# Santhosh-Sathyamurthy/cfd-simulations

Hardware: AMD Instinct MI355X
Metric: Gcell-updates/s on pressure-Poisson Jacobi; achieved HBM GB/s vs peak (higher is better)
Workload: dtype f32; 1 GPU; jacobi3d_7pt_1024x1024x1024_f32; decomposition=z-slab, halo=none, kernel_variant=0, waves=0, zchunk=0, temporal_blocking=0, tb_rows=0, rhs_workspace=True

## Files before the change

cfd-simulations_amd/csrc/jacobi3d_tbr.hip:

```cpp
#include <type_traits>

#include "internal.hpp"

namespace cfd {

namespace {

typedef float gv4g __attribute__((ext_vector_type(4)));
typedef const __attribute__((address_space(1))) gv4g *gcv4p;
typedef __attribute__((address_space(1))) gv4g *gv4p;
__device__ inline float4 ldg4(const float *p) {
    const gv4g v = *(gcv4p)p;
    return make_float4(v.x, v.y, v.z, v.w);
}
__device__ inline void stg4(float *p, float4 v) { *(gv4p)p = gv4g{v.x, v.y, v.z, v.w}; }
__device__ inline float4 lds4(const float *p) { return *reinterpret_cast<const float4 *>(p); }
__device__ inline void sts4(float *p, float4 v) { *reinterpret_cast<float4 *>(p) = v; }

typedef float gv4f __attribute__((ext_vector_type(4)));
typedef __attribute__((address_space(3))) void lds_void;
typedef __attribute__((address_space(3))) float lfloat;
typedef __attribute__((address_space(3))) gv4f lgv4f;
__device__ inline uint32_t lds_addr(const void *p) { return (uint32_t)(uintptr_t)(const lds_void *)p; }
__device__ inline lfloat *lds_ptr(uint32_t a) { return (lfloat *)(uintptr_t)a; }
__device__ inline float4 lds4l(const lfloat *p) {
    const gv4f v = *(const lgv4f *)p;
    return make_float4(v.x, v.y, v.z, v.w);
}
__device__ inline void sts4l(lfloat *p, float4 v) { *(lgv4f *)p = gv4f{v.x, v.y, v.z, v.w}; }
__device__ inline __amdgpu_buffer_rsrc_t plane_rsrc(const float *base, int p, int nz, size_t plane) {
    const bool in = p >= 0 && p <= nz - 1;
    return __builtin_amdgcn_make_buffer_rsrc(const_cast<float *>(in ? base + (size_t)p * plane : base),
                                             (short)0, in ? (int)(plane * sizeof(float)) : 0, 0x00020000);
}
constexpr int kStoreNt = 2;
#ifndef CFD_TBR_LB
#define CFD_TBR_LB 1
#endif
#ifndef CFD_TBR_XW
#define CFD_TBR_XW 1
#endif
#ifndef CFD_TBR_SD
#define CFD_TBR_SD 1
#endif
#ifndef CFD_TBR_T0S
#define CFD_TBR_T0S 1
#endif
#ifndef CFD_TBR_EARLY
#define CFD_TBR_EARLY 1
#endif


__device__ inline float4 ldb4(__amdgpu_buffer_rsrc_t r, uint32_t byte_ofs) {
    const gv4f v = __builtin_amdgcn_raw_buffer_load_b128(r, (int)byte_ofs, 0, 0);
    return make_float4(v.x, v.y, v.z, v.w);
}
__device__ inline v4i32 plane_rsrc4(const float *base, int p, int nz, size_t plane) {
    const bool in = p >= 0 && p <= nz - 1;
    const unsigned long long b = (unsigned long long)(in ? base + (size_t)p * plane : base);
    v4i32 r;
    r.x = __builtin_amdgcn_readfirstlane((int)(unsigned)b);
    r.y = __builtin_amdgcn_readfirstlane((int)((unsigned)(b >> 32) & 0xffffu));
    r.z = __builtin_amdgcn_readfirstlane(in ? (int)(plane * sizeof(float)) : 0);
    r.w = 0x00020000;
    return r;
}
__device__ inline void lds_barrier() { asm volatile("s_waitcnt lgkmcnt(0)\n\ts_barrier" ::: "memory"); }
enum { kJacobi = 0, kRbgs = 1 };
constexpr int sl3(int v) { return ((v % 3) + 3) % 3; }
constexpr int slk(int v, int k) { return ((v % k) + k) % k; }

struct TbrArgs {
    const float *in;
    float *out;
    const float *div;
    int nz, ny, nx, nseg, ntile_y, zb, ze, zchunk, fixed_lo, fixed_hi;
    float h2, dt;
    float cx, cy, cz, cd, dt_inv, tol;
    int zoff;
    int h0;
    float *maxc;
    int rollback;
    int nhalf;
    const int *count;
    int lag;
    float *rhs_out;
    int xbw;
    unsigned long long *trace;
};
constexpr int kTraceStep0 = 200, kTraceSteps = 64;
__device__ inline void trace_mark(unsigned long long *tr, int wave, int step, int e) {
#ifdef CFD_TBR_TRACE
    const int k = step - kTraceStep0;
    if (tr && blockIdx.x == 0 && (threadIdx.x & 63) == 0 && k >= 0 && k < kTraceSteps)
        tr[((size_t)wave * kTraceSteps + k) * 5 + e] = __builtin_readcyclecounter();
#else
    (void)tr;
    (void)wave;
    (void)step;
    (void)e;
#endif
}
enum { kFirstRhs = 1, kFirstZero = 2 };

template <int MODE, bool PRE, bool PK = false>
__device__ inline float4 level4(float4 c, float wl, float er, float4 N, float4 S, float4 U,
                                float4 D, float4 d, int x, int nx, bool upd, const TbrArgs &a,
                                int par, bool own, float &chg) {
    if (!upd) return c;
    if (MODE == kRbgs) {
        typedef float v2f __attribute__((ext_vector_type(2)));
        const bool hi = (par & 1) != 0;
        const v2f C = hi ? v2f{c.y, c.w} : v2f{c.x, c.z};
        const v2f E = hi ? v2f{c.z, er} : v2f{c.y, c.w};
        const v2f Wv = hi ? v2f{c.x, c.z} : v2f{wl, c.y};
        const v2f Nv = hi ? v2f{N.y, N.w} : v2f{N.x, N.z};
        const v2f Sv = hi ? v2f{S.y, S.w} : v2f{S.x, S.z};
        const v2f Uv = hi ? v2f{U.y, U.w} : v2f{U.x, U.z};
        const v2f Dv = hi ? v2f{D.y, D.w} : v2f{D.x, D.z};
        const v2f Rv = hi ? v2f{d.y, d.w} : v2f{d.x, d.z};
        const v2f rhs = -Rv * a.dt_inv;
        const v2f p = a.cx * (E + Wv);
        const v2f q = a.cy * (Nv + Sv);
        const v2f r = a.cz * (Uv + Dv);
        v2f o = (((p + q) + r) - rhs) * a.cd;
        const int x0 = x + (hi ? 1 : 0);
        o.x = (x0 != 0 && x0 != nx - 1) ? o.x : C.x;
        o.y = (x0 + 2 != nx - 1) ? o.y : C.y;
        if (own) {
            chg = fmaxf(chg, fabsf(o.x - C.x));
            chg = fmaxf(chg, fabsf(o.y - C.y));
        }
        return hi ? make_float4(c.x, o.x, c.z, o.y) : make_float4(o.x, c.y, o.y, c.w);
    }
    if constexpr (!PK) {
        float o[4];
        const float cv[4] = {c.x, c.y, c.z, c.w};
        const float nv[4] = {N.x, N.y, N.z, N.w};
        const float sv[4] = {S.x, S.y, S.z, S.w};
        const float uv[4] = {U.x, U.y, U.z, U.w};
        const float dv[4] = {D.x, D.y, D.z, D.w};
        const float rv[4] = {d.x, d.y, d.z, d.w};
#pragma unroll
        for (int k = 0; k < 4; ++k) {
            const float E = k < 3 ? cv[k + 1] : er;
            const float Wv = k > 0 ? cv[k - 1] : wl;
            float s = E + Wv;
            s = s + nv[k];
            s = s + sv[k];
            s = s + uv[k];
            s = s + dv[k];
            const float rhs = PRE ? rv[k] : (a.h2 * rv[k]) / a.dt;
            const int xk = x + k;
            o[k] = (xk != 0 && xk != nx - 1) ? (1.0f / 6.0f) * (s - rhs) : cv[k];
    }
    return make_float4(o[0], o[1], o[2], o[3]);
    }
    typedef float v2 __attribute__((ext_vector_type(2)));
    const v2 mid = {c.y, c.z};
    v2 s01 = mid + v2{wl, c.x};
    v2 s23 = v2{c.w, er} + mid;
    s01 = s01 + v2{N.x, N.y};
    s23 = s23 + v2{N.z, N.w};
    s01 = s01 + v2{S.x, S.y};
    s23 = s23 + v2{S.z, S.w};
    s01 = s01 + v2{U.x, U.y};
    s23 = s23 + v2{U.z, U.w};
    s01 = s01 + v2{D.x, D.y};
    s23 = s23 + v2{D.z, D.w};
    v2 r01 = {d.x, d.y}, r23 = {d.z, d.w};
    if constexpr (!PRE) {
        r01 = (a.h2 * r01) / a.dt;
        r23 = (a.h2 * r23) / a.dt;
    }
    v2 o01 = (1.0f / 6.0f) * (s01 - r01);
    v2 o23 = (1.0f / 6.0f) * (s23 - r23);
    o01.x = x != 0 ? o01.x : c.x;
    o23.y = x + 3 != nx - 1 ? o23.y : c.w;
    return make_float4(o01.x, o01.y, o23.x, o23.y);
}

typedef float v2f_t __attribute__((ext_vector_type(2)));
__device__ inline v2f_t pick2(float4 f, int h) { return h ? v2f_t{f.y, f.w} : v2f_t{f.x, f.z}; }
__device__ inline float4 join2(v2f_t a, v2f_t b, int h) {
    return h ? make_float4(b.x, a.x, b.y, a.y) : make_float4(a.x, b.x, a.y, b.y);
}
struct P4 {
    v2f_t e, o;
};
__device__ inline v2f_t pick2(const P4 &f, int h) { return h ? f.o : f.e; }
__device__ inline P4 split4(float4 f) { return P4{v2f_t{f.x, f.z}, v2f_t{f.y, f.w}}; }

#ifndef CFD_TBR_Q64
#define CFD_TBR_Q64 1
#endif
struct Q4 {
    unsigned long long lo, hi;
};
__device__ inline Q4 q4_of(float4 f) {
    return Q4{__builtin_bit_cast(unsigned long long, v2f_t{f.x, f.y}),
              __builtin_bit_cast(unsigned long long, v2f_t{f.z, f.w})};
}
__device__ inline float4 f4_of(const Q4 &q) {
    const v2f_t a = __builtin_bit_cast(v2f_t, q.lo), b = __builtin_bit_cast(v2f_t, q.hi);
    return make_float4(a.x, a.y, b.x, b.y);
}
[[maybe_unused]] __device__ inline float4 f4_of(float4 f) { return f; }
__device__ inline const P4 &f4_of(const P4 &p) { return p; }
__device__ inline P4 ldsp(const float *p) { return P4{v2f_t{p[0], p[2]}, v2f_t{p[1], p[3]}}; }
__device__ inline void sts4s(float *row, int lane, float4 v) {
    *reinterpret_cast<v2f_t *>(row + 4 + 2 * lane) = v2f_t{v.x, v.z};
    *reinterpret_cast<v2f_t *>(row + 132 + 2 * lane) = v2f_t{v.y, v.w};
}
__device__ inline void sts4s(float *row, int lane, const P4 &v) {
    *reinterpret_cast<v2f_t *>(row + 4 + 2 * lane) = v.e;
    *reinterpret_cast<v2f_t *>(row + 132 + 2 * lane) = v.o;
}
constexpr int kPairRow = 132;
__device__ inline v2f_t lds2s(const float *row, int lane, int h) {
    return *reinterpret_cast<const v2f_t *>(row + 4 + 128 * h + 2 * lane);
}
struct GsPk {
    v2f_t cx, cy, cz, cd, ndt;
};
__device__ inline GsPk gs_pk(const TbrArgs &a) {
    GsPk k{v2f_t{a.cx, a.cx}, v2f_t{a.cy, a.cy}, v2f_t{a.cz, a.cz}, v2f_t{a.cd, a.cd},
           v2f_t{-a.dt_inv, -a.dt_inv}};
    asm volatile("" : "+v"(k.cx), "+v"(k.cy), "+v"(k.cz), "+v"(k.cd), "+v"(k.ndt));
    return k;
}
__device__ inline v2f_t level2(v2f_t C, v2f_t O, float wl, float er, v2f_t N, v2f_t S, v2f_t U, v2f_t D,
                               v2f_t rhs, int h, int x, int nx, bool upd, const GsPk &a, bool own,
                               float &chg) {
    if (!upd) return C;
    const v2f_t E = h ? v2f_t{O.y, er} : v2f_t{O.x, O.y};
    const v2f_t W = h ? v2f_t{O.x, O.y} : v2f_t{wl, O.x};
    const v2f_t p = a.cx * (E + W);
    const v2f_t q = a.cy * (N + S);
    const v2f_t r = a.cz * (U + D);
    v2f_t o = (((p + q) + r) - rhs) * a.cd;
    const int x0 = x + h;
    if (h == 0) o.x = x0 != 0 ? o.x : C.x;
    if (h == 1) o.y = x0 + 2 != nx - 1 ? o.y : C.y;
    if (own) {
        chg = fmaxf(chg, fabsf(o.x - C.x));
        chg = fmaxf(chg, fabsf(o.y - C.y));
    }
    return o;
}

}

template <int K, int NWR, int RPW, bool PRE, int PD, int MODE, int F, bool SPLIT, bool PT, bool T0S = false>
__device__ __forceinline__ void tbr_halo_wave(const TbrArgs a, float *smem, int z0, int z1, int y0, int xs,
                                              int zl, float *slots = nullptr) {
    constexpr int NR = NWR * RPW + 2;
    constexpr int RS = 264, RS2 = kPairRow;
    int t0 = 0;
    auto T = [&](int l, int r) -> float * {
        if (T0S && l == 0) return slots + t0 + r * RS;
        int base = 0;
#pragma unroll
        for (int m = T0S ? 1 : 0; m < K; ++m)
            if (m < l) base += (NR - 2 * m) * (PT && m ? RS2 : RS);
        return smem + base + (r - l) * (PT && l ? RS2 : RS);
    };
    const int nz = a.nz, ny = a.ny, nx = a.nx;
    const int lane = threadIdx.x & 63;
    const int x = xs + 4 * lane;
    const bool xin = x < nx;
    const size_t plane = (size_t)ny * nx;
    const int zs = z0 - K + 1;
    auto P = [&](int p) { return a.in + (size_t)p * plane; };
    auto fixedp = [&](int p) { return (p == a.zb - 1 && a.fixed_lo) || (p == a.ze && a.fixed_hi); };
    const float4 z4 = make_float4(0.f, 0.f, 0.f, 0.f);
// ... 139 lines not shown
        return t;
    }();
    __shared__ __attribute__((aligned(16))) float smem[TOTAL > 0 ? TOTAL : 4];
    __shared__ __attribute__((aligned(16))) float slots[T0S ? 3 * SLOT : 4];
    constexpr int SR_ = NR - 2;
    constexpr int STG = T0S ? 3 * SLOT : 2 * SR_ * 256;
    constexpr bool DMA = PD == 1 && (TOTAL + STG) * 4 <= 160 * 1024;
    constexpr bool RDMA = DMA && (TOTAL + STG + 2 * SR_ * 256) * 4 <= 160 * 1024;
    static_assert(!T0S || DMA, "T0S: the LDS-DMA path");
    constexpr bool SPLIT = MODE == kRbgs && DMA;
    constexpr bool EARLY = DMA && MODE == kRbgs && CFD_TBR_EARLY;
    constexpr int SST = DMA && !T0S ? SR_ * 256 : 4;
    constexpr int SSR = RDMA ? SR_ * 256 : 4;
    __shared__ __attribute__((aligned(16))) float st_p0[SST], st_p1[SST], st_r0[SSR], st_r1[SSR];
    auto T = [&](int l, int r) -> float * {
        int base = 0;
#pragma unroll
        for (int m = T0S ? 1 : 0; m < K; ++m)
            if (m < l) base += (NR - 2 * m) * (PT && m ? RS2 : RS);
        return smem + base + (r - l) * (PT && l ? RS2 : RS);
    };

    static_assert(!PT || DMA, "pair tiles: LDS-DMA path");
    static_assert(MODE == kJacobi || !PRE, "GS: raw div");
    static_assert(F == 0 || (MODE == kJacobi && !PRE && DMA), "first pass: Jacobi, raw div, DMA path");
    constexpr bool ZERO = (F & kFirstZero) != 0, RHSW = (F & kFirstRhs) != 0;
    constexpr bool PREL = PRE || RHSW;
    auto torhs = [&](float4 d) {
        if constexpr (MODE == kRbgs) {
            d.x = -d.x * a.dt_inv;
            d.y = -d.y * a.dt_inv;
            d.z = -d.z * a.dt_inv;
            d.w = -d.w * a.dt_inv;
        }
        if constexpr (RHSW) {
            d.x = (a.h2 * d.x) / a.dt;
            d.y = (a.h2 * d.y) / a.dt;
            d.z = (a.h2 * d.z) / a.dt;
            d.w = (a.h2 * d.w) / a.dt;
        }
        return d;
    };
    constexpr int NIT = MODE == kRbgs ? (K + 2) / 2 : 1;
    if (MODE == kRbgs) {
        if (a.rollback) {
            const int P = a.rollback, H = 2 * *a.count;
            const int js = (H - 1) / P, need = H - P * js;
            if (need != K || need >= P || P * js + P > a.nhalf) return;
            a.h0 = P * js;
            if (js & 1) {
                float *t_ = const_cast<float *>(a.in);
                a.in = a.out;
                a.out = t_;
            }
        } else {
            const int ic = a.h0 >> 1, d = 1 + a.lag;
            if ((ic >= d && a.maxc[ic - d] < a.tol) || (ic >= d + 1 && a.maxc[ic - d - 1] < a.tol))
                return;
        }
    }
    const int nz = a.nz, ny = a.ny, nx = a.nx;
    const int lane = threadIdx.x & 63;
    const int wv = __builtin_amdgcn_readfirstlane(threadIdx.x >> 6);
    const int t = xcd_swizzle(blockIdx.x, gridDim.x);
    int seg = t % a.nseg;
    int ty = (t / a.nseg) % a.ntile_y;
    const int zc = t / (a.nseg * a.ntile_y);
    if (a.xbw) {
        const int per = gridDim.x / kNumXcd, x = t / per, k = t - x * per;
        const int nbx = a.nseg / a.xbw, bh = per / a.xbw;
        seg = (x % nbx) * a.xbw + k % a.xbw;
        ty = (x / nbx) * bh + k / a.xbw;
    }
    const int z0 = a.zb + zc * a.zchunk;
    if (z0 >= a.ze) return;
    const int z1 = min(z0 + a.zchunk, a.ze);
    const int y0 = 1 + ty * W;
    const int xs = seg * 256;
    const int x = xs + 4 * lane;
    const bool xin = x < nx;
    const size_t plane = (size_t)ny * nx;
    const int zs = z0 - K + 1;
    const int zl0 = z1 + K - 2;
    constexpr bool ROT = DMA && K <= 3 && (MODE == kJacobi || RPW <= 2) && !SHIFTQ;
    const int zl = ROT ? zs + 6 * ((zl0 - zs + 6) / 6) - 1 : zl0;
    auto P = [&](int p) { return a.in + (size_t)p * plane; };
    auto fixedp = [&](int p) { return (p == a.zb - 1 && a.fixed_lo) || (p == a.ze && a.fixed_hi); };
    const float4 z4 = make_float4(0.f, 0.f, 0.f, 0.f);
    constexpr int KS = MODE == kRbgs ? (K == 4 ? 2 : K) : 1;
    auto slot = [](int l) { return K == 4 ? (l - 1) >> 1 : l - 1; };
    float chgl[KS];
#pragma unroll
    for (int i = 0; i < KS; ++i) chgl[i] = 0.f;
    auto fold = [&](int l, float lm) {
        if constexpr (MODE == kRbgs) chgl[slot(l)] = fmaxf(chgl[slot(l)], lm);
    };

    if constexpr (T0S && ZERO) {
        for (int k = threadIdx.x; k < 3 * SLOT / 4; k += blockDim.x) sts4(slots + 4 * k, z4);
        __syncthreads();
    }
    if (wv < NWR) {
        if constexpr (DMA) {
            int rr[RPW];
            uint32_t bo[RPW], so[RPW];
            bool irow[RPW], orow[RPW];
#pragma unroll
            for (int j = 0; j < RPW; ++j) {
                rr[j] = 1 + wv + j * NWR;
                const int y = y0 - K + rr[j];
                const bool rowin = y >= 0 && y <= ny - 1;
                irow[j] = y >= 1 && y <= ny - 2;
                orow[j] = rr[j] >= K && rr[j] < NR - K && y <= ny - 2 && xin;
                const uint32_t o = (uint32_t)(((size_t)(rowin ? y : 0) * nx + (xin ? x : 0)) * sizeof(float));
                bo[j] = xin && rowin ? o : kOob;
                so[j] = orow[j] ? o : kOob;
            }
            using QT = std::conditional_t<MODE == kRbgs, v2f_t, float4>;
            using JQ = std::conditional_t<CFD_TBR_Q64 != 0, Q4, float4>;
            using VT = std::conditional_t<MODE == kRbgs, P4, JQ>;
            using QQ = std::conditional_t<MODE == kRbgs, v2f_t, JQ>;
            auto toV = [](float4 f) -> VT {
                if constexpr (MODE == kRbgs)
                    return split4(f);
                else if constexpr (CFD_TBR_Q64 != 0)
                    return q4_of(f);
                else
                    return f;
            };
            VT V[RPW][3], Rq[RPW][K];
            QQ Q[RPW][K][3];
            float4 Rn[RPW];
            constexpr bool LB = MODE == kJacobi && CFD_TBR_LB;
            constexpr int kTb2 = [] {
                int t = 0;
                for (int m = 0; m < 2 && m < K; ++m) t += (NR - 2 * m) * RS;
                return K >= 3 && !T0S ? t : 0;
            }();
            auto tbase = [](int l) {
                int t = 0;
                for (int m = T0S ? 1 : 0; m < l; ++m) t += (NR - 2 * m) * RS;
                return t;
            };
            [[maybe_unused]] const GsPk gk = MODE == kRbgs ? gs_pk(a) : GsPk{};
            const uint32_t lds_st_p0 = lds_addr(st_p0), lds_st_p1 = lds_addr(st_p1);
            const uint32_t lds_st_r0 = lds_addr(st_r0), lds_st_r1 = lds_addr(st_r1);
            (void)lds_st_p0;
            (void)lds_st_p1;
            (void)lds_st_r0;
            (void)lds_st_r1;
            const uint32_t lbA0 = lds_addr(smem) + 4u * (uint32_t)(wv * RS + 4 + 4 * lane);
            const uint32_t lbU0 = lds_addr(smem) + 4u * (uint32_t)(wv * RS);
            const uint32_t lbP00 = lds_addr(st_p0) + 4u * (uint32_t)(wv * 256 + 4 * lane);
            const uint32_t lbP10 = lds_addr(st_p1) + 4u * (uint32_t)(wv * 256 + 4 * lane);
            const uint32_t lbS0 = lds_addr(slots) + 4u * (uint32_t)(wv * RS + 4 + 4 * lane);
            const uint32_t lbUS0 = lds_addr(slots) + 4u * (uint32_t)(wv * RS);
            auto slot_row = [&](int q, int j) { return slots + q * SLOT + rr[j] * RS + 4; };
#pragma unroll
            for (int j = 0; j < RPW; ++j) {
#pragma unroll
                for (int l = 0; l < K; ++l) Q[j][l][0] = Q[j][l][1] = Q[j][l][2] = QQ{};
                V[j][ROT ? 2 : 0] = toV(ZERO ? z4 : ldb4(plane_rsrc(a.in, zs - 1, nz, plane), bo[j]));
                V[j][ROT ? 0 : 1] = toV(ZERO ? z4 : ldb4(plane_rsrc(a.in, zs, nz, plane), bo[j]));
                V[j][ROT ? 1 : 2] = toV(z4);
#pragma unroll
                for (int i = 0; i < K; ++i) Rq[j][i] = toV(z4);
                if constexpr (T0S) {
                    if (!ZERO) {
                        dma_row(plane_rsrc4(a.in, zs, nz, plane), bo[j], slot_row(0, j));
                        dma_row(plane_rsrc4(a.in, zs + 1, nz, plane), bo[j], slot_row(1, j));
                    }
                } else if (!ZERO) {
                    dma_row(plane_rsrc4(a.in, zs + 1, nz, plane), bo[j], st_p1 + (rr[j] - 1) * 256);
                }
                if constexpr (RDMA)
                    dma_row(plane_rsrc4(a.div, zs, nz, plane), bo[j], st_r1 + (rr[j] - 1) * 256);
                else
                    Rn[j] = ldb4(plane_rsrc(a.div, zs, nz, plane), bo[j]);
            }
            if constexpr (EARLY) {
#pragma unroll
                for (int j = 0; j < RPW; ++j) {
                    if (!ZERO) dma_row(plane_rsrc4(a.in, zs + 2, nz, plane), bo[j], st_p0 + (rr[j] - 1) * 256);
                    if constexpr (RDMA) dma_row(plane_rsrc4(a.div, zs + 1, nz, plane), bo[j], st_r0 + (rr[j] - 1) * 256);
                }
                wait_vmcnt<0>();
            }
            constexpr bool XW = MODE == kJacobi && !EARLY && CFD_TBR_XW;
            if constexpr (XW) wait_vmcnt<0>();
            constexpr bool ROTR = ROT && 6 % K == 0;
            constexpr int kND = ((ZERO ? 0 : 1) + (RDMA ? 1 : 0)) * RPW, kNR = RDMA ? 0 : RPW, kNSK = RPW,
                          kNSR = RHSW ? RPW : 0;
            static_assert(2 * kNSK + 2 * kNR + kNSR + kND < 64, "vmcnt range");
            constexpr bool SD = (XW || EARLY) && CFD_TBR_SD;
            constexpr int kAh = EARLY ? 3 : 2;
            const uint64_t pbytes = (uint64_t)plane * sizeof(float);
            uint64_t sd_in = (uint64_t)(uintptr_t)a.in + (uint64_t)(int64_t)(zs + kAh) * pbytes;
            uint64_t sd_div = (uint64_t)(uintptr_t)a.div + (uint64_t)(int64_t)(zs + kAh - 1) * pbytes;
            uint64_t sd_out = (uint64_t)(uintptr_t)a.out + (uint64_t)(int64_t)(zs - K + 1) * pbytes;
            uint64_t sd_rhs = (uint64_t)(uintptr_t)a.rhs_out + (uint64_t)(int64_t)zs * pbytes;
            int sd_oz = 0, sd_on = 4 * SLOT, sd_od = 8 * SLOT;
            const int sd_flo = a.fixed_lo ? a.zb - 1 : -(1 << 30), sd_fhi = a.fixed_hi ? a.ze : -(1 << 30);
            auto rsrc4 = [&](uint64_t b, bool ok) {
                v4i32 r;
                r.x = __builtin_amdgcn_readfirstlane((int)(uint32_t)b);
                r.y = __builtin_amdgcn_readfirstlane((int)((uint32_t)(b >> 32) & 0xffffu));
                r.z = __builtin_amdgcn_readfirstlane(ok ? (int)pbytes : 0);
                r.w = 0x00020000;
                return r;
            };
            auto rsrc = [&](uint64_t b, bool ok) {
                return __builtin_amdgcn_make_buffer_rsrc((void *)(uintptr_t)b, (short)0, ok ? (int)pbytes : 0,
                                                         0x00020000);
            };
            (void)rsrc4;
            (void)rsrc;
            auto step = [&](int z, auto parc, auto rotc, auto bpc) {
                constexpr int E = decltype(parc)::value;
                constexpr int R = decltype(rotc)::value;
                auto vs = [](int d) { return ROT ? sl3(R + d) : d + 1; };
                auto qs = [](int l, int d) { return ROT ? sl3(R - l - 1 + d) : d; };
                constexpr int BPv = decltype(bpc)::value;
                trace_mark(a.trace, wv, z - zs, 0);
                float *const pw = E ? st_p1 : st_p0;
                float *const rw = E ? st_r1 : st_r0;
                const float *const pr = E ? st_p0 : st_p1;
                const float *const rdr = E ? st_r0 : st_r1;
                const int sz = T0S && !SD ? (z - zs) % 3 : 0;
                const int sn = sz == 2 ? 0 : sz + 1, sd = sn == 2 ? 0 : sn + 1;
                const uint32_t oz = SD ? (uint32_t)sd_oz : 4u * (uint32_t)(sz * SLOT);
                const uint32_t on = SD ? (uint32_t)sd_on : 4u * (uint32_t)(sn * SLOT);
                const uint32_t od = SD ? (uint32_t)sd_od : 4u * (uint32_t)(sd * SLOT);
                uint32_t bA = lbA0, bU = lbU0, bP = E ? lbP00 : lbP10;
                uint32_t bS = lbS0 + oz, bSn = lbS0 + on;
                uint32_t bUS = lbUS0 + oz;
                if constexpr (LB && T0S)
                    asm volatile("" : "+v"(bA), "+v"(bU), "+v"(bS), "+v"(bSn), "+v"(bUS));
                else if constexpr (LB)
                    asm volatile("" : "+v"(bA), "+v"(bU), "+v"(bP));
                const uint32_t bB = bA + 4u * kTb2, bUB = bU + 4u * kTb2;
                auto tp = [&](int l, int d) -> lfloat * {
                    if (T0S && l == 0) return lds_ptr(bS) + (1 + d) * RS;
                    return l < 2 ? lds_ptr(bA) + (tbase(l) + (1 + d - l) * RS)
                                 : lds_ptr(bB) + (tbase(l) - kTb2 + (1 + d - l) * RS);
                };
                auto up = [&](int l, int d) -> const lfloat * {
                    if (T0S && l == 0) return lds_ptr(bUS) + (1 + d) * RS;
                    return l < 2 ? lds_ptr(bU) + (tbase(l) + (1 + d - l) * RS)
                                 : lds_ptr(bUB) + (tbase(l) - kTb2 + (1 + d - l) * RS);
                };
                (void)sd;
                (void)tp;
                (void)up;
                float4 Rc[RPW];
                if constexpr (!RDMA && XW) {
#pragma unroll
                    for (int j = 0; j < RPW; ++j) Rc[j] = Rn[j];
                }
                if constexpr (!EARLY) {
                    const v4i32 rp = SD ? rsrc4(sd_in, z + 2 >= 0 && z + 2 <= nz - 1) : plane_rsrc4(a.in, z + 2, nz, plane);
                    const v4i32 rd = SD ? rsrc4(sd_div, z + 1 >= 0 && z + 1 <= nz - 1) : plane_rsrc4(a.div, z + 1, nz, plane);
#pragma unroll
                    for (int j = 0; j < RPW; ++j) {
                        if (!ZERO)
                            dma_row(rp, bo[j],
                                    T0S ? (SD ? (float *)((char *)slots + od) + rr[j] * RS + 4 : slot_row(sd, j))
                                        : pw + (rr[j] - 1) * 256);
                        if constexpr (RDMA) dma_row(rd, bo[j], rw + (rr[j] - 1) * 256);
                    }
                } else {
                    (void)pw;
                    (void)rw;
                }
                if constexpr (!RDMA) {
                    (void)rw;
                    (void)rdr;
                    const __amdgpu_buffer_rsrc_t rdn =
                        SD ? rsrc(sd_div - (EARLY ? pbytes : 0), z + 1 >= 0 && z + 1 <= nz - 1)
                           : plane_rsrc(a.div, z + 1, nz, plane);
#pragma unroll
                    for (int j = 0; j < RPW; ++j) {
                        if constexpr (!XW) Rc[j] = Rn[j];
                        Rn[j] = ldb4(rdn, bo[j]);
                    }
                }
#pragma unroll
                for (int j = 0; j < RPW; ++j) {
                    if (xin && !T0S) {
                        if constexpr (SPLIT)
                            sts4s(T(0, rr[j]), lane, f4_of(V[j][vs(0)]));
                        else if constexpr (LB)
                            sts4l(tp(0, j * NWR), f4_of(V[j][vs(0)]));
                        else
                            sts4(T(0, rr[j]) + 4 + 4 * lane, f4_of(V[j][vs(0)]));
                    }
#pragma unroll
                    for (int l = 1; l < K; ++l)
                        if (xin && rr[j] >= l && rr[j] < NR - l) {
                            if constexpr (MODE == kRbgs) {
                                const int h = (BPv ^ E ^ (j * NWR)) & 1;
                                const v2f_t lo = l == 1 ? pick2(V[j][vs(-1)], h)
                                                        : Q[j][l - 1][ROT ? sl3(R - l) : 1];
                                if constexpr (PT) {
                                    (void)lo;
                                    *reinterpret_cast<v2f_t *>(T(l, rr[j]) + 2 + 2 * lane) =
                                        Q[j][l][ROT ? sl3(R - l) : 2];
                                } else {
                                    const float4 f = join2(lo, Q[j][l][ROT ? sl3(R - l) : 2], h);
                                    if constexpr (SPLIT)
                                        sts4s(T(l, rr[j]), lane, f);
                                    else
                                        sts4(T(l, rr[j]) + 4 + 4 * lane, f);
                                }
                            } else if constexpr (LB) {
                                sts4l(tp(l, j * NWR), f4_of(Q[j][l][ROT ? sl3(R - l) : 2]));
                            } else {
                                sts4(T(l, rr[j]) + 4 + 4 * lane, f4_of(Q[j][l][ROT ? sl3(R - l) : 2]));
                            }
                        }
                }
                if constexpr (EARLY)
                    wait_vmcnt<2 * kNSK + 2 * kNR + kNSR + kND>();
                else if constexpr (XW)
                    wait_vmcnt<2 * kNR + kNSR + kND>();
                else
                    wait_vmcnt<((ZERO ? 0 : 1) + 1) * RPW>();
                trace_mark(a.trace, wv, z - zs, 1);
                lds_barrier();
                trace_mark(a.trace, wv, z - zs, 2);
#pragma unroll
                for (int j = 0; j < RPW; ++j) {
                    if constexpr (MODE == kRbgs)
                        V[j][vs(1)] = ldsp(pr + (rr[j] - 1) * 256 + 4 * lane);
                    else if constexpr (LB && T0S)
                        V[j][vs(1)] = toV(ZERO ? z4 : lds4l(lds_ptr(bSn) + (1 + j * NWR) * RS));
                    else if constexpr (LB)
                        V[j][vs(1)] = toV(ZERO ? z4 : lds4l(lds_ptr(bP) + j * NWR * 256));
                    else
                        V[j][vs(1)] = toV(ZERO ? z4 : lds4(pr + (rr[j] - 1) * 256 + 4 * lane));
                    constexpr int RS0 = ROTR ? slk(R, K) : 0;
                    if constexpr (!ROTR) {
#pragma unroll
                        for (int i = K - 1; i > 0; --i) Rq[j][i] = Rq[j][i - 1];
                    }
                    if constexpr (RDMA && MODE == kRbgs) {
                        P4 d = ldsp(rdr + (rr[j] - 1) * 256 + 4 * lane);
                        d.e = d.e * gk.ndt;
                        d.o = d.o * gk.ndt;
                        Rq[j][RS0] = d;
                    } else if constexpr (RDMA) {
                        Rq[j][RS0] = toV(torhs(lds4(rdr + (rr[j] - 1) * 256 + 4 * lane)));
                    } else {
                        Rq[j][RS0] = toV(torhs(Rc[j]));
                    }
                    if constexpr (RHSW) {
                        const bool own = z >= z0 && z < z1;
                        const __amdgpu_buffer_rsrc_t ro =
                            SD ? rsrc(sd_rhs, own)
                               : __builtin_amdgcn_make_buffer_rsrc(a.rhs_out + (size_t)(own ? z : 0) * plane, (short)0,
                                                                   own ? (int)(plane * sizeof(float)) : 0, 0x00020000);
                        const float4 rq = f4_of(Rq[j][RS0]);
                        const gv4f rv = {rq.x, rq.y, rq.z, rq.w};
                        __builtin_amdgcn_raw_buffer_store_b128(rv, ro, (int)so[j], 0, kStoreNt);
                    }
                }
                if constexpr (EARLY) {
                    asm volatile("s_waitcnt lgkmcnt(0)" ::: "memory");
                    const v4i32 rp = SD ? rsrc4(sd_in, z + 3 >= 0 && z + 3 <= nz - 1) : plane_rsrc4(a.in, z + 3, nz, plane);
                    const v4i32 rd = SD ? rsrc4(sd_div, z + 2 >= 0 && z + 2 <= nz - 1) : plane_rsrc4(a.div, z + 2, nz, plane);
                    const uint32_t lpr = E ? lds_st_p0 : lds_st_p1, lrr = E ? lds_st_r0 : lds_st_r1;
#pragma unroll
                    for (int j = 0; j < RPW; ++j) {
                        const uint32_t ro_ = 1024u * (uint32_t)(rr[j] - 1);
                        if (!ZERO) dma_row_at(rp, bo[j], lpr + ro_);
                        if constexpr (RDMA) dma_row_at(rd, bo[j], lrr + ro_);
                    }
                }
                struct LdsIn {
                    QT N, S;
                    float wl, er;
                };
                auto fetch = [&](int l, int j) {
                    const int r = rr[j];
                    LdsIn o;
                    const float *row = T(l - 1, r);
                    if constexpr (MODE == kRbgs) {
                        const int h = (BPv ^ E ^ (j * NWR)) & 1;
                        const bool pt = PT && l > 1;
                        o.wl = pt ? row[1] : row[3];
                        o.er = pt ? row[130] : row[260];
                        if (pt) {
                            o.N = *reinterpret_cast<const v2f_t *>(T(l - 1, r + 1) + 2 + 2 * lane);
                            o.S = *reinterpret_cast<const v2f_t *>(T(l - 1, r - 1) + 2 + 2 * lane);
                        } else if (SPLIT) {
                            o.N = lds2s(T(l - 1, r + 1), lane, h);
                            o.S = lds2s(T(l - 1, r - 1), lane, h);
                        } else {
                            o.N = pick2(lds4(T(l - 1, r + 1) + 4 + 4 * lane), h);
                            o.S = pick2(lds4(T(l - 1, r - 1) + 4 + 4 * lane), h);
                        }
                    } else if constexpr (LB) {
                        (void)row;
                        o.wl = up(l - 1, j * NWR)[3];
                        o.er = up(l - 1, j * NWR)[260];
                        o.N = lds4l(tp(l - 1, j * NWR + 1));
                        o.S = lds4l(tp(l - 1, j * NWR - 1));
                    } else {
                        o.wl = row[3];
                        o.er = row[260];
                        o.N = lds4(T(l - 1, r + 1) + 4 + 4 * lane);
                        o.S = lds4(T(l - 1, r - 1) + 4 + 4 * lane);
                    }
                    return o;
                };
#pragma unroll
                for (int l = 1; l <= K; ++l) {
                    const int p = z - l + 1;
                    const bool fx = SD ? ((p == sd_flo) | (p == sd_fhi)) : fixedp(p);
                    if (!RDMA && XW && l == K) {
#pragma unroll
                        for (int j = 0; j < RPW; ++j) {
                            gv4f r4 = {Rn[j].x, Rn[j].y, Rn[j].z, Rn[j].w};
                            asm volatile("" : "+v"(r4));
                            Rn[j] = make_float4(r4.x, r4.y, r4.z, r4.w);
                        }
                    }
#pragma unroll
                    for (int j = 0; j < RPW; ++j) {
                        const int r = rr[j];
                        if constexpr (MODE == kRbgs) {
                          if (r >= l && r < NR - l) {
                            const int h = (BPv ^ E ^ (j * NWR)) & 1;
                            const v2f_t Cp = l == 1   ? pick2(V[j][vs(0)], h)
                                             : l == 2 ? pick2(V[j][vs(-1)], h)
                                                      : Q[j][l - 2][qs(l - 2, 0)];
                            const v2f_t Op = l == 1 ? pick2(V[j][vs(0)], 1 - h) : Q[j][l - 1][qs(l - 1, 1)];
                            const v2f_t Up = l == 1 ? pick2(V[j][vs(1)], h) : Q[j][l - 1][qs(l - 1, 2)];
                            const v2f_t Dp = l == 1 ? pick2(V[j][vs(-1)], h) : Q[j][l - 1][qs(l - 1, 0)];
                            const LdsIn in = fetch(l, j);
                            const float wl = dpp_from_lower_old(in.wl, Op.y), er = dpp_from_upper_old(in.er, Op.x);
                            const v2f_t v = level2(Cp, Op, wl, er, in.N, in.S, Up, Dp,
                                                   pick2(Rq[j][ROTR ? slk(R - l + 1, K) : l - 1], h), h, x, nx,
                                                   irow[j] && !fx, gk, orow[j] && p >= z0 && p < z1, chgl[slot(l)]);
                            if (l < K) {
                                if constexpr (ROT) {
                                    Q[j][l][sl3(R - l + 1)] = v;
                                } else {
                                    Q[j][l][0] = Q[j][l][1];
                                    Q[j][l][1] = Q[j][l][2];
                                    Q[j][l][2] = v;
                                }
                            } else {
                                const float4 f = join2(v, Op, h);
                                const bool own = p >= z0 && p < z1;
                                const __amdgpu_buffer_rsrc_t ro =
                                    SD ? rsrc(sd_out, own)
                                       : __builtin_amdgcn_make_buffer_rsrc(a.out + (size_t)(own ? p : 0) * plane,
                                                                           (short)0,
                                                                           own ? (int)(plane * sizeof(float)) : 0,
                                                                           0x00020000);
                                const gv4f vv = {f.x, f.y, f.z, f.w};
                                __builtin_amdgcn_raw_buffer_store_b128(vv, ro, (int)so[j], 0, kStoreNt);
                            }
                          }
                        } else if (r >= l && r < NR - l) {
                            const float4 c = f4_of(l == 1 ? V[j][vs(0)] : Q[j][l - 1][qs(l - 1, 1)]);
                            const float4 U = f4_of(l == 1 ? V[j][vs(1)] : Q[j][l - 1][qs(l - 1, 2)]);
                            const float4 D = f4_of(l == 1 ? V[j][vs(-1)] : Q[j][l - 1][qs(l - 1, 0)]);
                            const LdsIn in = fetch(l, j);
                            const float wl = dpp_from_lower_old(in.wl, c.w);
                            const float er = dpp_from_upper_old(in.er, c.x);
                            float lm = 0.f;
                            const float4 v = level4<MODE, PREL, K == 4>(c, wl, er, in.N, in.S, U, D,
                                                                f4_of(Rq[j][ROTR ? slk(R - l + 1, K) : l - 1]), x, nx,
                                                                irow[j] && !fx, a, (BPv ^ E ^ (j * NWR)) & 1,
                                                                orow[j] && p >= z0 && p < z1, lm);
                            fold(l, lm);
                            if (l < K) {
                                if constexpr (ROT) {
                                    Q[j][l][sl3(R - l + 1)] = toV(v);
                                } else {
                                    Q[j][l][0] = Q[j][l][1];
                                    Q[j][l][1] = Q[j][l][2];
                                    Q[j][l][2] = toV(v);
                                }
                            } else {
                                const bool own = p >= z0 && p < z1;
                                const __amdgpu_buffer_rsrc_t ro =
                                    SD ? rsrc(sd_out, own)
                                       : __builtin_amdgcn_make_buffer_rsrc(a.out + (size_t)(own ? p : 0) * plane,
                                                                           (short)0,
                                                                           own ? (int)(plane * sizeof(float)) : 0,
                                                                           0x00020000);
                                const gv4f vv = {v.x, v.y, v.z, v.w};
                                __builtin_amdgcn_raw_buffer_store_b128(vv, ro, (int)so[j], 0, kStoreNt);
                            }
                        }
                        if (EARLY && l == K && !(r >= l && r < NR - l)) {
                            const __amdgpu_buffer_rsrc_t ro =
                                __builtin_amdgcn_make_buffer_rsrc(a.out, (short)0, 0, 0x00020000);
                            __builtin_amdgcn_raw_buffer_store_b128(gv4f{0.f, 0.f, 0.f, 0.f}, ro, (int)kOob, 0, kStoreNt);
                        }
                        if constexpr (K <= 3) __builtin_amdgcn_sched_barrier(0);
                    }
                }
                trace_mark(a.trace, wv, z - zs, 3);
                lds_barrier();
                trace_mark(a.trace, wv, z - zs, 4);
                if constexpr (SD) {
                    sd_in += pbytes;
                    sd_div += pbytes;
                    sd_out += pbytes;
                    sd_rhs += pbytes;
                    const int t_ = sd_oz;
                    sd_oz = sd_on;
                    sd_on = sd_od;
                    sd_od = t_;
                }
                if constexpr (!ROT) {
#pragma unroll
                    for (int j = 0; j < RPW; ++j) {
                        V[j][0] = V[j][1];
                        V[j][1] = V[j][2];
                    }
                }
            };
            using I0 = std::integral_constant<int, 0>;
            using I1 = std::integral_constant<int, 1>;
            auto march = [&](auto bpc) {
                if constexpr (!ROT) {
                    for (int zb = zs; zb <= zl; zb += 2) {
                        step(zb, I0{}, I0{}, bpc);
                        if (zb + 1 <= zl) step(zb + 1, I1{}, I0{}, bpc);
                    }
                    return;
                }
                for (int zb = zs; zb <= zl; zb += 6) {
                    step(zb, std::integral_constant<int, 0>{}, std::integral_constant<int, 0>{}, bpc);
                    step(zb + 1, std::integral_constant<int, 1>{}, std::integral_constant<int, 1>{}, bpc);
                    step(zb + 2, std::integral_constant<int, 0>{}, std::integral_constant<int, 2>{}, bpc);
                    step(zb + 3, std::integral_constant<int, 1>{}, std::integral_constant<int, 3>{}, bpc);
                    step(zb + 4, std::integral_constant<int, 0>{}, std::integral_constant<int, 4>{}, bpc);
                    step(zb + 5, std::integral_constant<int, 1>{}, std::integral_constant<int, 5>{}, bpc);
                }
            };
            if (MODE == kRbgs && ((a.zoff + zs + y0 + K + wv + a.h0) & 1))
                march(std::integral_constant<int, 1>{});
            else
                march(std::integral_constant<int, 0>{});
            wait_vmcnt<0>();
        } else {
            int rr[RPW];
            size_t ofs[RPW];
            bool ld[RPW], irow[RPW], orow[RPW];
#pragma unroll
            for (int j = 0; j < RPW; ++j) {
                rr[j] = 1 + wv + j * NWR;
                const int y = y0 - K + rr[j];
                const bool rowin = y >= 0 && y <= ny - 1;
                ld[j] = xin && rowin;
                irow[j] = y >= 1 && y <= ny - 2;
                orow[j] = rr[j] >= K && rr[j] < NR - K && y <= ny - 2 && xin;
                ofs[j] = (size_t)(rowin ? y : 0) * nx + (xin ? x : 0);
            }
            auto ldp = [&](int j, int p) {
                return (ld[j] && p >= 0 && p <= nz - 1) ? ldg4(P(p) + ofs[j]) : z4;
            };
            auto ldr = [&](int j, int p) {
                return (ld[j] && p >= 0 && p <= nz - 1) ? ldg4(a.div + (size_t)p * plane + ofs[j]) : z4;
            };
            float4 Q[RPW][K][3];
            float4 Rq[RPW][K];
            float4 Cq[RPW][PD], Rn[RPW][PD];
#pragma unroll
            for (int j = 0; j < RPW; ++j) {
#pragma unroll
                for (int l = 0; l < K; ++l) Q[j][l][0] = Q[j][l][1] = Q[j][l][2] = z4;
                Q[j][0][0] = ldp(j, zs - 1);
                Q[j][0][1] = ldp(j, zs);
                Q[j][0][2] = ldp(j, zs + 1);
#pragma unroll
                for (int i = 0; i < K; ++i) Rq[j][i] = ldr(j, zs - i);
#pragma unroll
                for (int i = 0; i + 1 < PD; ++i) {
                    Cq[j][i] = ldp(j, zs + 2 + i);
                    Rn[j][i] = ldr(j, zs + 1 + i);
                }
            }
            for (int z = zs; z <= zl; ++z) {
#pragma unroll
                for (int j = 0; j < RPW; ++j) {
                    Cq[j][PD - 1] = ldp(j, z + 1 + PD);
                    Rn[j][PD - 1] = ldr(j, z + PD);
                }
#pragma unroll
                for (int j = 0; j < RPW; ++j) {
                    if (ld[j]) sts4(T(0, rr[j]) + 4 + 4 * lane, Q[j][0][1]);
#pragma unroll
                    for (int l = 1; l < K; ++l)
                        if (xin && rr[j] >= l && rr[j] < NR - l) sts4(T(l, rr[j]) + 4 + 4 * lane, Q[j][l][2]);
                }
                __syncthreads();
#pragma unroll
                for (int l = 1; l <= K; ++l) {
                    const int p = z - l + 1;
                    const bool fx = fixedp(p);
#pragma unroll
                    for (int j = 0; j < RPW; ++j) {
                        const int r = rr[j];
                        if (r >= l && r < NR - l) {
                            const float4 c = Q[j][l - 1][1];
                            float wl = __shfl_up(c.w, 1, 64);
                            float er = __shfl_down(c.x, 1, 64);
                            const float *row = T(l - 1, r);
                            const float wl_l = row[3], er_l = row[260];
                            if (lane == 0) wl = wl_l;
// ... 73 lines not shown
                                {2, 10, 2, true}, {2, 10, 3, false}, {2, 9, 2, true}, {1, 9, 2, true}};

int num_cus() {
    static int n = 0;
    if (n <= 0) {
        int dev = 0;
        if (hipGetDevice(&dev) != hipSuccess ||
            hipDeviceGetAttribute(&n, hipDeviceAttributeMultiprocessorCount, dev) != hipSuccess || n <= 0)
            n = 256;
    }
    return n;
}
thread_local int g_cu_reserve = 0;
thread_local int g_last_shape[4] = {0, 0, 0, 0};
}

int tbr_cus() { return num_cus() - g_cu_reserve; }
void set_cu_reserve(int n) { g_cu_reserve = n; }

template <int MODE>
static int tbr_launch(TbrArgs a, int K, int rows, int zchunk, bool pre, hipStream_t s, int first = 0) {
    const int pd = jacobi3d_tb_prefetch();
    if (first && (MODE != kJacobi || pre || pd != 1 || rows != 0 || K < 2)) {
        set_error("jacobi3d_tbr: a first pass needs Jacobi, raw div, prefetch 1, auto tiles, 2..4 levels");
        return CFD_E_INVALID;
    }
    if (a.nx % 4 != 0) {
        set_error("jacobi3d_tbr: nx must be a multiple of 4");
        return CFD_E_INVALID;
    }
    const int L = a.ze - a.zb;
    const int nseg = ceil_div(a.nx, 256);
    const int ncu = tbr_cus();
    const TbrShape *best = nullptr;
    int best_zlen = 0;
    double best_cost = 0.0;
    for (const TbrShape &sh : kShapes) {
        if (sh.K != K || (rows ? sh.rows() != rows : !sh.autopick)) continue;
        const int W = sh.rows(), NR = W + 2 * K;
        const long tiles = (long)nseg * ceil_div(a.ny - 2, W);
        for (int nzc = 1; nzc <= 64; ++nzc) {
            int zlen = zchunk > 0 ? zchunk : ceil_div(L, nzc);
            if (zlen > L) zlen = L;
            if (zchunk <= 0 && zlen < 8 && L >= 8) break;
            const long wgs = tiles * ceil_div(L, zlen);
            const double cost = (double)ceil_div(wgs, ncu) * (zlen + 2 * K - 2 + 8) * NR;
            if (!best || cost < best_cost) {
                best = &sh;
                best_cost = cost;
                best_zlen = zlen;
            }
            if (zchunk > 0) break;
        }
    }
    if (!best) {
        set_error("jacobi3d_tbr: no tile shape with %d rows for %d levels per pass", rows, K);
        return CFD_E_INVALID;
    }
    a.nseg = nseg;
    a.ntile_y = ceil_div(a.ny - 2, best->rows());
    a.trace = reinterpret_cast<unsigned long long *>(tuning().tbr_trace);
    a.zchunk = best_zlen;
    {
        static const int xbw_env = [] {
            const char *e = getenv("CFD_TBR_XBW");
            return e ? atoi(e) : 0;
        }();
        const int tiles = nseg * a.ntile_y, per = tiles / kNumXcd;
        a.xbw = 0;
        if (xbw_env > 0 && best_zlen >= L && tiles % kNumXcd == 0 && nseg % xbw_env == 0 && per % xbw_env == 0 &&
            (kNumXcd / (nseg / xbw_env)) * (per / xbw_env) == a.ntile_y && kNumXcd % (nseg / xbw_env) == 0)
            a.xbw = xbw_env;
    }
    g_last_shape[0] = best->K;
    g_last_shape[1] = best->nwr;
    g_last_shape[2] = best->rpw;
    g_last_shape[3] = best_zlen;
    const int blocks = a.nseg * a.ntile_y * ceil_div(L, best_zlen);
    const int nsteps = best_zlen + 2 * best->K - 2;
    static const bool shiftq_all = [] {
        const char *e = getenv("CFD_TBR_SHIFTQ");
        return e && atoi(e) == 1;
    }();
    const bool shiftq = MODE == kJacobi && pd == 1 && best->K == 3 &&
                        (shiftq_all || (nsteps % 6 != 0 && nsteps < 216));
#define CFD_TBR_L(KV, NW, RP, PR, PDV) \
    hipLaunchKernelGGL((jacobi3d_tbr<KV, NW, RP, PR, PDV, MODE>), dim3(blocks), dim3((NW + 1) * 64), 0, s, a)
#define CFD_TBR(KV, NW, RP)                                                                   \
    do {                                                                                      \
        if constexpr (MODE == kRbgs) {                                                        \
            if (pd == 2) CFD_TBR_L(KV, NW, RP, false, 2); else CFD_TBR_L(KV, NW, RP, false, 1); \
        } else if (pd == 2) {                                                                 \
            if (pre) CFD_TBR_L(KV, NW, RP, true, 2); else CFD_TBR_L(KV, NW, RP, false, 2);      \
        } else {                                                                              \
            if (pre) CFD_TBR_L(KV, NW, RP, true, 1); else CFD_TBR_L(KV, NW, RP, false, 1);      \
        }                                                                                     \
    } while (0)
#define CFD_TBRF(KV, NW, RP)                                                                 \
    do {                                                                                     \
        if constexpr (MODE == kJacobi && KV == 3) {                                          \
            if (shiftq) {                                                                    \
                if (first == (kFirstRhs | kFirstZero))                                       \
                    hipLaunchKernelGGL((jacobi3d_tbr<KV, NW, RP, false, 1, MODE, kFirstRhs | kFirstZero, true>), \
                                       dim3(blocks), dim3((NW + 1) * 64), 0, s, a);          \
                else if (first == kFirstRhs)                                                 \
                    hipLaunchKernelGGL((jacobi3d_tbr<KV, NW, RP, false, 1, MODE, kFirstRhs, true>), \
                                       dim3(blocks), dim3((NW + 1) * 64), 0, s, a);          \
                else if (pre)                                                                \
                    hipLaunchKernelGGL((jacobi3d_tbr<KV, NW, RP, true, 1, MODE, 0, true>),   \
                                       dim3(blocks), dim3((NW + 1) * 64), 0, s, a);          \
                else                                                                         \
                    hipLaunchKernelGGL((jacobi3d_tbr<KV, NW, RP, false, 1, MODE, 0, true>),  \
                                       dim3(blocks), dim3((NW + 1) * 64), 0, s, a);          \
                break;                                                                       \
            }                                                                                \
        }                                                                                    \
        if constexpr (MODE == kJacobi) {                                                     \
            if (first == (kFirstRhs | kFirstZero)) {                                         \
                hipLaunchKernelGGL((jacobi3d_tbr<KV, NW, RP, false, 1, MODE, kFirstRhs | kFirstZero>), \
                                   dim3(blocks), dim3((NW + 1) * 64), 0, s, a);              \
                break;                                                                       \
            }                                                                                \
            if (first == kFirstRhs) {                                                        \
                hipLaunchKernelGGL((jacobi3d_tbr<KV, NW, RP, false, 1, MODE, kFirstRhs>),     \
                                   dim3(blocks), dim3((NW + 1) * 64), 0, s, a);              \
                break;                                                                       \
            }                                                                                \
        }                                                                                    \
        CFD_TBR(KV, NW, RP);                                                                 \
    } while (0)
    const int code = best->K * 100 + best->nwr * 10 + best->rpw;
    if (first && code != 3 * 100 + 11 * 10 + 2 && code != 3 * 100 + 10 * 10 + 2 &&
        code != 4 * 100 + 11 * 10 + 2 && code != 2 * 100 + 11 * 10 + 2 && code != 2 * 100 + 10 * 10 + 2 &&
        code != 2 * 100 + 9 * 10 + 2) {
        set_error("jacobi3d_tbr: tile shape (%d levels, %d x %d rows) has no first-pass variant", best->K,
                  best->nwr, best->rpw);
        return CFD_E_INVALID;
    }
    switch (code) {
        case 3 * 100 + 11 * 10 + 2: CFD_TBRF(3, 11, 2); break;
        case 3 * 100 + 10 * 10 + 2: CFD_TBRF(3, 10, 2); break;
        case 1 * 100 + 9 * 10 + 2: if constexpr (MODE == kRbgs) CFD_TBR(1, 9, 2); break;
        case 3 * 100 + 7 * 10 + 3: if constexpr (MODE == kJacobi) CFD_TBR(3, 7, 3); break;
        case 4 * 100 + 7 * 10 + 3: CFD_TBR(4, 7, 3); break;
        case 4 * 100 + 11 * 10 + 2: CFD_TBRF(4, 11, 2); break;
        case 4 * 100 + 10 * 10 + 2: CFD_TBR(4, 10, 2); break;
        case 2 * 100 + 11 * 10 + 2: CFD_TBRF(2, 11, 2); break;
        case 2 * 100 + 10 * 10 + 2: CFD_TBRF(2, 10, 2); break;
        case 2 * 100 + 9 * 10 + 2: CFD_TBRF(2, 9, 2); break;
        default: CFD_TBR(2, 10, 3); break;
    }
#undef CFD_TBRF
#undef CFD_TBR
#undef CFD_TBR_L
    CFD_LAUNCH_CHECK();
    return CFD_OK;
}

int jacobi3d_tbr_pass(int K, int rows, const float *in, float *out, const float *div, int nz,
                      int ny, int nx, int zb, int ze, int fixed_lo, int fixed_hi, float h2,
                      float dt, int zchunk, bool pre, hipStream_t s) {
    if (ze <= zb || ny < 3) return CFD_OK;
    TbrArgs a{};
    a.in = in; a.out = out; a.div = div;
    a.nz = nz; a.ny = ny; a.nx = nx; a.zb = zb; a.ze = ze;
    a.fixed_lo = fixed_lo; a.fixed_hi = fixed_hi; a.h2 = h2; a.dt = dt;
    return tbr_launch<kJacobi>(a, K, rows, zchunk, pre, s);
}

int jacobi3d_tbr_first_pass(int K, float *out, const float *div, float *rhs_out, const float *in,
                            int nz, int ny, int nx, int zb, int ze, int fixed_lo, int fixed_hi,
                            float h2, float dt, int zchunk, bool zero, hipStream_t s) {
    if (ze <= zb || ny < 3) return CFD_OK;
    TbrArgs a{};
    a.in = zero ? out : in; a.out = out; a.div = div; a.rhs_out = rhs_out;
    a.nz = nz; a.ny = ny; a.nx = nx; a.zb = zb; a.ze = ze;
    a.fixed_lo = fixed_lo; a.fixed_hi = fixed_hi; a.h2 = h2; a.dt = dt;
    return tbr_launch<kJacobi>(a, K, 0, zchunk, false, s, kFirstRhs | (zero ? kFirstZero : 0));
}

int rbgs3d_tbr_pass(const float *in, float *out, const float *div, int nz, int ny, int nx, int zb,
                    int ze, int fixed_lo, int fixed_hi, int zoff, const RbgsConsts &k, int h0,
                    int levels, RbgsWs *ws, int rollback, int nhalf, int rows, hipStream_t s,
// ... 27 lines not shown
```

Baseline: 1735 Gcell-updates/s.

## Add period-3 register rotation for K=4 temporal-blocked Jacobi kernel

Extends the rotating register-slot scheme to K=4, RPW=2 configurations with a period-3 z-loop unroll, so plane queues rotate by index instead of being copied. Under the V1 option the level-1 centre and upper planes are read straight from LDS and only the lower plane is kept in registers, which cuts register pressure. It also enables the shift-queue variant for K=4 when the step count pads badly to a multiple of three. The trade-off is extra LDS reads and up to two padded steps at the end of each chunk.

```diff
diff --git a/cfd-simulations_amd/csrc/jacobi3d_tbr.hip b/cfd-simulations_amd/csrc/jacobi3d_tbr.hip
--- a/cfd-simulations_amd/csrc/jacobi3d_tbr.hip
+++ b/cfd-simulations_amd/csrc/jacobi3d_tbr.hip
@@ -48,6 +48,12 @@
 #endif
 #ifndef CFD_TBR_EARLY
 #define CFD_TBR_EARLY 1
+#endif
+#ifndef CFD_TBR_ROT3
+#define CFD_TBR_ROT3 1
+#endif
+#ifndef CFD_TBR_V1
+#define CFD_TBR_V1 1
 #endif
 
 
@@ -191,6 +197,11 @@
 __device__ inline v2f_t pick2(const P4 &f, int h) { return h ? f.o : f.e; }
 __device__ inline P4 split4(float4 f) { return P4{v2f_t{f.x, f.z}, v2f_t{f.y, f.w}}; }
 
+__device__ inline float4 any4() {
+    gv4f v;
+    asm volatile("" : "=v"(v));
+    return make_float4(v.x, v.y, v.z, v.w);
+}
 #ifndef CFD_TBR_Q64
 #define CFD_TBR_Q64 1
 #endif
@@ -496,8 +507,10 @@
     const size_t plane = (size_t)ny * nx;
     const int zs = z0 - K + 1;
     const int zl0 = z1 + K - 2;
-    constexpr bool ROT = DMA && K <= 3 && (MODE == kJacobi || RPW <= 2) && !SHIFTQ;
-    const int zl = ROT ? zs + 6 * ((zl0 - zs + 6) / 6) - 1 : zl0;
+    constexpr bool ROT3 = T0S && K == 4 && RPW == 2 && !RDMA && !SHIFTQ && CFD_TBR_ROT3;
+    constexpr bool ROT = (DMA && K <= 3 && (MODE == kJacobi || RPW <= 2) && !SHIFTQ) || ROT3;
+    constexpr int PER = ROT3 ? 3 : 6;
+    const int zl = ROT ? zs + PER * ((zl0 - zs + PER) / PER) - 1 : zl0;
     auto P = [&](int p) { return a.in + (size_t)p * plane; };
     auto fixedp = [&](int p) { return (p == a.zb - 1 && a.fixed_lo) || (p == a.ze && a.fixed_hi); };
     const float4 z4 = make_float4(0.f, 0.f, 0.f, 0.f);
@@ -542,6 +555,7 @@
                 else
                     return f;
             };
+            constexpr bool V1 = ROT3 && CFD_TBR_V1;
             VT V[RPW][3], Rq[RPW][K];
             QQ Q[RPW][K][3];
             float4 Rn[RPW];
@@ -574,9 +588,11 @@
             for (int j = 0; j < RPW; ++j) {
 #pragma unroll
                 for (int l = 0; l < K; ++l) Q[j][l][0] = Q[j][l][1] = Q[j][l][2] = QQ{};
-                V[j][ROT ? 2 : 0] = toV(ZERO ? z4 : ldb4(plane_rsrc(a.in, zs - 1, nz, plane), bo[j]));
-                V[j][ROT ? 0 : 1] = toV(ZERO ? z4 : ldb4(plane_rsrc(a.in, zs, nz, plane), bo[j]));
-                V[j][ROT ? 1 : 2] = toV(z4);
+                V[j][V1 ? 0 : ROT ? 2 : 0] = toV(ZERO ? z4 : ldb4(plane_rsrc(a.in, zs - 1, nz, plane), bo[j]));
+                if constexpr (!V1) {
+                    V[j][ROT ? 0 : 1] = toV(ZERO ? z4 : ldb4(plane_rsrc(a.in, zs, nz, plane), bo[j]));
+                    V[j][ROT ? 1 : 2] = toV(z4);
+                }
 #pragma unroll
                 for (int i = 0; i < K; ++i) Rq[j][i] = toV(z4);
                 if constexpr (T0S) {
@@ -602,7 +618,7 @@
             }
             constexpr bool XW = MODE == kJacobi && !EARLY && CFD_TBR_XW;
             if constexpr (XW) wait_vmcnt<0>();
-            constexpr bool ROTR = ROT && 6 % K == 0;
+            constexpr bool ROTR = ROT && PER % K == 0;
             constexpr int kND = ((ZERO ? 0 : 1) + (RDMA ? 1 : 0)) * RPW, kNR = RDMA ? 0 : RPW, kNSK = RPW,
                           kNSR = RHSW ? RPW : 0;
             static_assert(2 * kNSK + 2 * kNR + kNSR + kND < 64, "vmcnt range");
@@ -746,6 +762,8 @@
                 for (int j = 0; j < RPW; ++j) {
                     if constexpr (MODE == kRbgs)
                         V[j][vs(1)] = ldsp(pr + (rr[j] - 1) * 256 + 4 * lane);
+                    else if constexpr (V1)
+                        ;
                     else if constexpr (LB && T0S)
                         V[j][vs(1)] = toV(ZERO ? z4 : lds4l(lds_ptr(bSn) + (1 + j * NWR) * RS));
                     else if constexpr (LB)
@@ -877,10 +895,21 @@
                                 __builtin_amdgcn_raw_buffer_store_b128(vv, ro, (int)so[j], 0, kStoreNt);
                             }
                           }
-                        } else if (r >= l && r < NR - l) {
-                            const float4 c = f4_of(l == 1 ? V[j][vs(0)] : Q[j][l - 1][qs(l - 1, 1)]);
-                            const float4 U = f4_of(l == 1 ? V[j][vs(1)] : Q[j][l - 1][qs(l - 1, 2)]);
-                            const float4 D = f4_of(l == 1 ? V[j][vs(-1)] : Q[j][l - 1][qs(l - 1, 0)]);
+                        } else if ((ROT3 && l == 1) || (r >= l && r < NR - l)) {
+                            float4 c, U, D;
+                            if constexpr (V1) {
+                                if (l == 1) {
+                                    c = ZERO ? z4 : lds4l(tp(0, j * NWR));
+                                    U = ZERO ? z4 : lds4l(lds_ptr(bSn) + (1 + j * NWR) * RS);
+                                    D = f4_of(V[j][0]);
+                                    V[j][0] = toV(c);
+                                }
+                            }
+                            if (!V1 || l > 1) {
+                                c = f4_of(l == 1 ? V[j][vs(0)] : Q[j][l - 1][qs(l - 1, 1)]);
+                                U = f4_of(l == 1 ? V[j][vs(1)] : Q[j][l - 1][qs(l - 1, 2)]);
+                                D = f4_of(l == 1 ? V[j][vs(-1)] : Q[j][l - 1][qs(l - 1, 0)]);
+                            }
                             const LdsIn in = fetch(l, j);
                             const float wl = dpp_from_lower_old(in.wl, c.w);
                             const float er = dpp_from_upper_old(in.er, c.x);
@@ -909,6 +938,8 @@
                                 const gv4f vv = {v.x, v.y, v.z, v.w};
                                 __builtin_amdgcn_raw_buffer_store_b128(vv, ro, (int)so[j], 0, kStoreNt);
                             }
+                        } else if constexpr (ROT3) {
+                            if (l < K) Q[j][l][sl3(R - l + 1)] = toV(any4());
                         }
                         if (EARLY && l == K && !(r >= l && r < NR - l)) {
                             const __amdgpu_buffer_rsrc_t ro =
@@ -946,6 +977,14 @@
                     for (int zb = zs; zb <= zl; zb += 2) {
                         step(zb, I0{}, I0{}, bpc);
                         if (zb + 1 <= zl) step(zb + 1, I1{}, I0{}, bpc);
+                    }
+                    return;
+                }
+                if constexpr (ROT3) {
+                    for (int zb = zs; zb <= zl; zb += 3) {
+                        step(zb, I0{}, std::integral_constant<int, 0>{}, bpc);
+                        step(zb + 1, I0{}, std::integral_constant<int, 1>{}, bpc);
+                        step(zb + 2, I0{}, std::integral_constant<int, 2>{}, bpc);
                     }
                     return;
                 }
@@ -1185,8 +1224,10 @@
         const char *e = getenv("CFD_TBR_SHIFTQ");
         return e && atoi(e) == 1;
     }();
-    const bool shiftq = MODE == kJacobi && pd == 1 && best->K == 3 &&
-                        (shiftq_all || (nsteps % 6 != 0 && nsteps < 216));
+    const int extra3 = (3 - nsteps % 3) % 3;
+    const bool shiftq = MODE == kJacobi && pd == 1 &&
+                        ((best->K == 3 && (shiftq_all || (nsteps % 6 != 0 && nsteps < 216))) ||
+                         (best->K == 4 && (shiftq_all || nsteps < 48 * extra3)));
 #define CFD_TBR_L(KV, NW, RP, PR, PDV) \
     hipLaunchKernelGGL((jacobi3d_tbr<KV, NW, RP, PR, PDV, MODE>), dim3(blocks), dim3((NW + 1) * 64), 0, s, a)
 #define CFD_TBR(KV, NW, RP)                                                                   \
@@ -1201,7 +1242,7 @@
     } while (0)
 #define CFD_TBRF(KV, NW, RP)                                                                 \
     do {                                                                                     \
-        if constexpr (MODE == kJacobi && KV == 3) {                                          \
+        if constexpr (MODE == kJacobi && (KV == 3 || KV == 4)) {                             \
             if (shiftq) {                                                                    \
                 if (first == (kFirstRhs | kFirstZero))                                       \
                     hipLaunchKernelGGL((jacobi3d_tbr<KV, NW, RP, false, 1, MODE, kFirstRhs | kFirstZero, true>), \
```

Measured after the change: 1771 Gcell-updates/s, median of 6. +2.1%, better.
